# shidanxu/DistributedLPSolver

Measured on AMD Instinct MI355X. Metric: simplex pivots/s + achieved HBM GB/s (dense fp64 tableau; roofline of the rank-64 tableau pass), higher is better.
Workload: dtype f64

## Files before the change

distributedlpsolver_amd/csrc/dlp_pass.hip:

```cpp
#include <hip/hip_runtime.h>

#include <cmath>
#include <cstdlib>
#include <algorithm>
#include <type_traits>
#include <utility>

#include "dlp_host.h"
#include "dlp_internal.h"

namespace dlp {
namespace {

#include "dlp_device.h"
#include "dlp_defer_device.h"

constexpr int kUntouched = -3, kDense = -2, kSparse = -1;

template <int K>
__device__ inline d2 chain_dense(d2 t, const d2* pr, const double* nf) {
#pragma unroll
    for (int l = 0; l < K; ++l) {
        t.x = __builtin_fma(nf[l], pr[l].x, t.x);
        t.y = __builtin_fma(nf[l], pr[l].y, t.y);
// ... 519 lines not shown
#pragma unroll
                for (int u = 0; u < U; ++u)
#pragma unroll
                    for (int e = 0; e < V; ++e)
                        t[u][e] = __builtin_fma(-f[u][l], pr[l0 + l][e], t[u][e]);
    };
    auto grow = [&](int g) { return (int)__builtin_amdgcn_readfirstlane(dgl[g]) * U; };
    const __amdgpu_buffer_rsrc_t rs = __builtin_amdgcn_make_buffer_rsrc(
        (void*)(T + i0 * ld), (short)0, (int)((int64_t)nr * ld * 8), 0x00020000);
    const int voff = (int)(jc * 8);
    const int ld8 = (int)(ld * 8);
    auto load = [&](double (&t)[U][V], int r0) {
#pragma unroll
        for (int u = 0; u < U; ++u) bld<NT, V>(t[u], rs, voff, (r0 + u) * ld8);
    };
    auto store = [&](const double (&t)[U][V], int r0) {
#pragma unroll
        for (int u = 0; u < U; ++u) bst<NT, V>(t[u], rs, voff, (r0 + u) * ld8);
    };
    double fa[U][LC], fb[U][LC];
    auto group_full = [&](double (&t)[U][V], int r0, int rn) {
        const cdptr cb = (cdptr)(cbase + (int64_t)r0 * ldc);
        const cdptr cn = (cdptr)(cbase + (int64_t)rn * ldc);
#pragma unroll
        for (int c = 0; c < NCH; c += 2) {
            __builtin_amdgcn_s_waitcnt(0xC07F);
            fetch(fb, cb, (c + 1) * LC);
            __builtin_amdgcn_sched_barrier(0);
            chain(t, fa, c * LC);
            __builtin_amdgcn_sched_barrier(0);
            __builtin_amdgcn_s_waitcnt(0xC07F);
            if (c + 2 < NCH)
                fetch(fa, cb, (c + 2) * LC);
            else
                fetch(fa, cn, 0);
            __builtin_amdgcn_sched_barrier(0);
            chain(t, fb, (c + 1) * LC);
            __builtin_amdgcn_sched_barrier(0);
        }
        store(t, r0);
    };
    auto group_part = [&](double (&t)[U][V], int r0) {
        const cdptr cb = (cdptr)(cbase + (int64_t)r0 * ldc);
        fetch(fa, cb, 0);
#pragma unroll
        for (int c = 0; c < NCH; c += 2) {
            if (c * LC < kb) {
                __builtin_amdgcn_s_waitcnt(0xC07F);
                if ((c + 1) * LC < kb) fetch(fb, cb, (c + 1) * LC);
                __builtin_amdgcn_sched_barrier(0);
                if ((c + 1) * LC <= kb)
                    chain(t, fa, c * LC);
                else
                    chain_part(t, fa, c * LC);
                __builtin_amdgcn_sched_barrier(0);
                if ((c + 1) * LC < kb) {
                    __builtin_amdgcn_s_waitcnt(0xC07F);
                    if ((c + 2) * LC < kb && c + 2 < NCH) fetch(fa, cb, (c + 2) * LC);
                    __builtin_amdgcn_sched_barrier(0);
                    if ((c + 2) * LC <= kb)
                        chain(t, fb, (c + 1) * LC);
                    else
                        chain_part(t, fb, (c + 1) * LC);
                    __builtin_amdgcn_sched_barrier(0);
                }
            }
        }
        store(t, r0);
    };

    if (ndg > 0) {
        double buf[D][U][V];
#pragma unroll
        for (int b = 0; b < D - 1; ++b) load(buf[b], grow(b < ndg ? b : ndg - 1));
        if constexpr (!PART) fetch(fa, (cdptr)(cbase + (int64_t)grow(0) * ldc), 0);
        for (int g0 = 0; g0 < ndg; g0 += D) {
#pragma unroll
            for (int b = 0; b < D; ++b) {
                const int gi = g0 + b;
                if (gi < ndg) {
                    const int ga = gi + D - 1 < ndg ? gi + D - 1 : ndg - 1;
                    load(buf[(b + D - 1) % D], grow(ga));
                    __builtin_amdgcn_sched_barrier(0);
                    if constexpr (!PART)
                        group_full(buf[b], grow(gi), grow(gi + 1 < ndg ? gi + 1 : gi));
                    else
                        group_part(buf[b], grow(gi));
                }
            }
        }
    }
    for (int r = 0; r < nr; ++r) {
        const int c = cls[r];
        if (c == kUntouched) continue;
        const double* cr = C + (i0 + r) * ldc;
        double t[V];
        int l = 0;
        if (c >= 0) {
            ldrow<false, V>(t, P + (int64_t)c * ld + jc);
            l = c + 1;
        } else {
            bld<NT, V>(t, rs, voff, r * ld8);
        }
        for (; l < kb; ++l) {
            const double f = cr[l];
            if (f != 0.0) {
                double pv[V];
                ldrow<false, V>(pv, P + (int64_t)l * ld + jc);
#pragma unroll
                for (int e = 0; e < V; ++e) t[e] = __builtin_fma(-f, pv[e], t[e]);
            }
        }
        bst<NT, V>(t, rs, voff, r * ld8);
    }
}


constexpr int kDensePiv = 64;
__device__ inline void classify_band(int32_t* cls, const BlockDesc* __restrict__ bd,
                                     const int32_t* __restrict__ nzc, int64_t i0, int nr, int kb,
                                     bool densepiv = false) {
    for (int r = threadIdx.x; r < nr; r += blockDim.x) {
        const int nz = nzc[i0 + r];
        cls[r] = kb == 0 || nz == 0 ? kUntouched : (nz == kb ? kDense : kSparse);
    }
    __syncthreads();
    for (int l = threadIdx.x; l < kb; l += blockDim.x) {
        const int64_t r = (int64_t)bd->pl[l] - i0;
        if (bd->pl[l] >= 0 && r >= 0 && r < nr) atomicMax(&cls[r], l);
    }
    if (!densepiv) return;
    __syncthreads();
    for (int l = threadIdx.x; l < kb; l += blockDim.x) {
        const int64_t r = (int64_t)bd->pl[l] - i0;
        if (bd->pl[l] >= 0 && r >= 0 && r < nr && cls[r] == l && nzc[i0 + r] == kb) cls[r] = kDensePiv + l;
    }
}

template <int N>
__device__ __forceinline__ void fmac_bc(double& t, double c, double p) {
    asm("v_fmac_f64_dpp %0, -%1, %2 row_newbcast:%3 row_mask:0xf bank_mask:0xf"
        : "+v"(t)
        : "v"(c), "v"(p), "n"(N));
}
template <int N>
__device__ __forceinline__ double bc_mov(double v) {
    return __builtin_amdgcn_update_dpp(0.0, v, 0x150 + N, 0xf, 0xf, false);
}
template <int L>
__device__ __forceinline__ void dpp_step(double (&t)[2], const double (&c)[2][2][2], const double (&pr)[64]) {
    constexpr int h = L / 32, e = L & 1, n = (L & 31) >> 1;
    fmac_bc<n>(t[0], c[0][h][e], pr[L]);
    fmac_bc<n>(t[1], c[1][h][e], pr[L]);
}
template <int L0, int... I>
__device__ __forceinline__ void dpp_half(double (&t)[2], const double (&c)[2][2][2], const double (&pr)[64],
                                         std::integer_sequence<int, I...>) {
    (dpp_step<L0 + I>(t, c, pr), ...);
}

template <typename F>
__device__ __forceinline__ double replay_row(double t, int cl, const double (&pr)[64], F f) {
#pragma unroll
    for (int l = 0; l < 64; ++l) {
        const double c = f(l);
        if (l == cl)
            t = pr[l];
        else if (l > cl && c != 0.0)
            t = __builtin_fma(-c, pr[l], t);
    }
    return t;
}

template <bool NT, bool PUB = false>
__global__ __launch_bounds__(256) void pass_d_kernel(const double* __restrict__ T, double* __restrict__ Tout,
                                                     int64_t ld, int64_t rows, int64_t width,
                                                     const BlockDesc* __restrict__ bd,
                                                     const double* __restrict__ C, int64_t ldc,
                                                     const double* __restrict__ P,
                                                     const int32_t* __restrict__ nzc, int rb,
                                                     uint32_t* bcnt = nullptr) {
    constexpr int K = 64, U = 2;
    constexpr int kSt = (NT ? 2 : 0) | (PUB ? kAuxSc1 : 0);
    __shared__ int32_t cls[1024];
    const int kb = bd->blk;
    const bool outplace = Tout != T;
    if (kb == 0 && !outplace) return;
    const int64_t j = (int64_t)blockIdx.x * 256 + threadIdx.x;
    const bool colok = j < width;
    const int jc = (int)(colok ? j : width - 1);
    double pr[K];
#pragma unroll
    for (int l = 0; l < K; ++l) pr[l] = P[(int64_t)l * ld + jc];
    const int64_t i0 = (int64_t)blockIdx.y * rb;
    const int64_t iend = (i0 + rb < rows) ? i0 + rb : rows;
    const int nr = (int)(iend - i0);
    classify_band(cls, bd, nzc, i0, nr, kb);
    __syncthreads();
    const int ld8 = (int)(ld * 8);
    const __amdgpu_buffer_rsrc_t rt = __builtin_amdgcn_make_buffer_rsrc(
        (void*)(T + i0 * ld), (short)0, (int)((int64_t)nr * ld * 8), 0x00020000);
    const __amdgpu_buffer_rsrc_t ro = __builtin_amdgcn_make_buffer_rsrc(
        (void*)(Tout + i0 * ld), (short)0, (int)((int64_t)nr * ld * 8), 0x00020000);
    const __amdgpu_buffer_rsrc_t rc = __builtin_amdgcn_make_buffer_rsrc(
        (void*)(C + i0 * ldc), (short)0, (int)((int64_t)nr * ldc * 8), 0x00020000);
    const int voff = jc * 8;
    const int soff_bad = 0x7fffff00;
    const int voff_st = colok ? voff : soff_bad;
    const int coff = (threadIdx.x & 15) * 16;
    auto dense_at = [&](int r0) {
        if (r0 + U > nr) return false;
        return cls[r0] == kDense && cls[r0 + 1] == kDense;
    };
    double c[U][2][2];
    auto loadc = [&](int r0, int h) {
#pragma unroll
        for (int u = 0; u < U; ++u) {
            const u4v x = __builtin_amdgcn_raw_buffer_load_b128(rc, coff + h * 256, (r0 + u) * (int)ldc * 8, 0);
            const d2 v = __builtin_bit_cast(d2, x);
            c[u][h][0] = v.x;
            c[u][h][1] = v.y;
        }
    };
    auto loadt = [&](double (&t)[U], int r0) {
#pragma unroll
        for (int u = 0; u < U; ++u) {
            const u2v x = __builtin_amdgcn_raw_buffer_load_b64(rt, voff, (r0 + u) * ld8, NT ? 2 : 0);
            t[u] = __builtin_bit_cast(double, x);
        }
    };
    auto group = [&](double (&t)[U], double (&tn)[U], int r0, int rn) {
        loadt(tn, rn);
        __builtin_amdgcn_sched_barrier(0);
        dpp_half<0>(t, c, pr, std::make_integer_sequence<int, 32>{});
        __builtin_amdgcn_sched_barrier(0);
        loadc(rn, 0);
        __builtin_amdgcn_sched_barrier(0);
        dpp_half<32>(t, c, pr, std::make_integer_sequence<int, 32>{});
        __builtin_amdgcn_sched_barrier(0);
        loadc(rn, 1);
        __builtin_amdgcn_sched_barrier(0);
#pragma unroll
        for (int u = 0; u < U; ++u)
            __builtin_amdgcn_raw_buffer_store_b64(__builtin_bit_cast(u2v, t[u]), ro, voff_st, (r0 + u) * ld8,
                                                  kSt);
    };
    double ta[U], tb[U];
    int r = 0;
    while (r < nr) {
        if (dense_at(r)) {
            loadt(ta, r);
            loadc(r, 0);
            loadc(r, 1);
            while (true) {
                const bool nb = dense_at(r + U);
                group(ta, tb, r, nb ? r + U : r);
                r += U;
                if (!nb) break;
                const bool na = dense_at(r + U);
                group(tb, ta, r, na ? r + U : r);
                r += U;
                if (!na) break;
            }
            continue;
        }
        const int cl = cls[r];
        if (cl == kUntouched && outplace) {
            const u2v x = __builtin_amdgcn_raw_buffer_load_b64(rt, voff, r * ld8, NT ? 2 : 0);
            __builtin_amdgcn_raw_buffer_store_b64(x, ro, voff_st, r * ld8, kSt);
        } else if (cl != kUntouched) {
            const double* cr = C + (i0 + r) * ldc;
            double t = 0.0;
            if (cl < 0)
                t = __builtin_bit_cast(double, __builtin_amdgcn_raw_buffer_load_b64(rt, voff, r * ld8, NT ? 2 : 0));
            t = replay_row(t, cl, pr, [&](int l) { return cr[l]; });
            __builtin_amdgcn_raw_buffer_store_b64(__builtin_bit_cast(u2v, t), ro, voff_st, r * ld8, kSt);
        }
        r += 1;
    }
    if constexpr (PUB) {
        asm volatile("s_waitcnt vmcnt(0)" ::: "memory");
        __syncthreads();
        if (threadIdx.x == 0) __hip_atomic_fetch_add(&bcnt[blockIdx.y], 1u, __ATOMIC_RELAXED, __HIP_MEMORY_SCOPE_AGENT);
    }
}

template <int D, int U>
__device__ __forceinline__ void vmwait_group(int g) {
    static_assert(D <= 8 && 2 * U * (D - 1) <= 63, "vmcnt holds 6 bits");
    if (g >= D - 1) {
        vmwait<2 * U * (D - 1)>();
        return;
    }
    switch (g) {
        case 0: vmwait<U * (D - 1)>(); break;
        case 1: vmwait<U * (D - 1) + U>(); break;
        case 2: vmwait<U * (D - 1) + 2 * U>(); break;
        case 3: vmwait<U * (D - 1) + 3 * U>(); break;
        case 4: vmwait<U * (D - 1) + 4 * U>(); break;
        case 5: vmwait<U * (D - 1) + 5 * U>(); break;
        default: vmwait<U * (D - 1) + 6 * U>(); break;
    }
}
template <int U, int L>
__device__ __forceinline__ void ring_step(double (&t)[U], const double (&c)[U][2], const double (&pr)[64]) {
    constexpr int e = L & 1, n = (L & 31) >> 1;
#pragma unroll
    for (int u = 0; u < U; ++u) fmac_bc<n>(t[u], c[u][e], pr[L]);
}
template <int U, int L0, int... I>
__device__ __forceinline__ void ring_half(double (&t)[U], const double (&c)[U][2], const double (&pr)[64],
                                          std::integer_sequence<int, I...>) {
    (ring_step<U, L0 + I>(t, c, pr), ...);
}

template <int L>
__device__ __forceinline__ void redo_step(double& t, const double (&c)[2], const double (&pr)[64], int cl) {
    constexpr int e = L & 1, n = (L & 31) >> 1;
    if (L == cl)
        t = pr[L];
    else if (L > cl)
        fmac_bc<n>(t, c[e], pr[L]);
}
template <int L0, int... I>
__device__ __forceinline__ void redo_half(double& t, const double (&c)[2], const double (&pr)[64], int cl,
                                          std::integer_sequence<int, I...>) {
    (redo_step<L0 + I>(t, c, pr, cl), ...);
}
__device__ __forceinline__ double redo_pivot_row(const double* cr, int cl, const double (&pr)[64]) {
    int lane;
    asm volatile("v_mbcnt_lo_u32_b32 %0, -1, 0\n\tv_mbcnt_hi_u32_b32 %0, -1, %0" : "=v"(lane));
    double t = 0.0;
    if (cl < 32) {
        const d2 v = *(const d2*)(cr + 2 * (lane & 15));
        const double c0[2] = {v.x, v.y};
        redo_half<0>(t, c0, pr, cl, std::make_integer_sequence<int, 32>{});
    }
    const d2 v = *(const d2*)(cr + 32 + 2 * (lane & 15));
    const double c1[2] = {v.x, v.y};
    redo_half<32>(t, c1, pr, cl, std::make_integer_sequence<int, 32>{});
    return t;
}

template <bool NT, int U, int D, bool SA = false, bool PUB = false>
__global__ __launch_bounds__(256) __attribute__((amdgpu_waves_per_eu(3))) void pass_q_kernel(
                                                     const double* __restrict__ T, double* __restrict__ Tout,
                                                     int64_t ld, int64_t rows, int64_t width,
                                                     const BlockDesc* __restrict__ bd,
                                                     const double* __restrict__ C, int64_t ldc,
                                                     const double* __restrict__ P,
                                                     const int32_t* __restrict__ nzc, int rb,
                                                     uint32_t* bcnt = nullptr, int pivg = 0) {
    constexpr int K = 64, SLOT = 128 * U;
    constexpr int kSt = (NT ? 2 : 0) | (PUB ? kAuxSc1 : 0);
    static_assert(U % 2 == 0, "one DMA carries two rows");
    __shared__ __attribute__((aligned(16))) int32_t cls[1024];
    typedef int32_t clsv __attribute__((ext_vector_type(U)));
    extern __shared__ double ring[];
    const int kb = bd->blk;
    const bool outplace = Tout != T;
    if (kb == 0 && !outplace) return;
    const int lane = threadIdx.x & 63;
    const int w = __builtin_amdgcn_readfirstlane(threadIdx.x >> 6);
    const int64_t j = (int64_t)blockIdx.x * 256 + threadIdx.x;
    const bool colok = j < width;
    const int jc = (int)(colok ? j : width - 1);
    double pr[K];
#pragma unroll
    for (int l = 0; l < K; ++l) pr[l] = P[(int64_t)l * ld + jc];
    const int64_t i0 = (int64_t)blockIdx.y * rb;
    const int64_t iend = (i0 + rb < rows) ? i0 + rb : rows;
    const int nr = (int)(iend - i0);
    classify_band(cls, bd, nzc, i0, nr, kb, pivg != 0);
    __syncthreads();
#pragma unroll
    for (int l = 0; l < K; ++l) asm volatile("" ::"v"(pr[l]));
    const int ng = (nr + U - 1) / U;
    const int64_t wc = (int64_t)blockIdx.x * 256 + w * 64 + 2 * (lane & 31);
    const int64_t wcc = wc < ld - 1 ? wc : ld - 2;
    double* wbase = ring + (size_t)w * D * SLOT;
    const uint32_t lbase = (uint32_t)(uintptr_t)(const __attribute__((address_space(3))) void*)wbase;
    uint32_t tvoff = 0, cvoff = 0;
    const double *tsrc = nullptr, *csrc = nullptr;
    if constexpr (SA) {
        tvoff = (uint32_t)(lane >> 5) * (uint32_t)(ld * 8) + (uint32_t)(wcc * 8);
        cvoff = 16u * lane;
    } else {
        tsrc = T + i0 * ld + wcc;
        csrc = C + i0 * ldc + 2 * (lane & 31);
    }
    auto dma = [&](int g, int s) {
        const int gg = g < ng ? g : ng - 1;
#pragma unroll
        for (int k = 0; k < U / 2; ++k) {
            const uint32_t m0 = __builtin_amdgcn_readfirstlane(lbase + s * SLOT * 8 + k * 1024);
            if constexpr (SA) {
                const int rk = gg * U + 2 * k;
                const bool pair = rk + 1 < nr;
                const uint32_t up = lane >> 5 ? (uint32_t)(ld * 8) : 0u;
                glds16s(pair ? tvoff : tvoff - up, T + (i0 + (rk < nr ? rk : nr - 1)) * ld, m0);
            } else {
                int r = gg * U + 2 * k + (lane >> 5);
                r = r < nr ? r : nr - 1;
                glds16(tsrc + (int64_t)r * ld, m0);
            }
        }
#pragma unroll
        for (int k = 0; k < U / 2; ++k) {
            const uint32_t m0 = __builtin_amdgcn_readfirstlane(lbase + s * SLOT * 8 + U * 512 + k * 1024);
            if constexpr (SA) {
                const int rk = gg * U + 2 * k;
                const bool pair = rk + 1 < nr;
                glds16s(pair ? cvoff : cvoff & 511u, C + (i0 + (rk < nr ? rk : nr - 1)) * ldc, m0);
            } else {
                int r = gg * U + 2 * k + (lane >> 5);
                r = r < nr ? r : nr - 1;
                glds16(csrc + (int64_t)r * ldc, m0);
            }
        }
    };
    const int ngs = SA ? nr / U : 0;
    const int64_t tstep = (int64_t)U * ld * 8, cstep = (int64_t)U * ldc * 8;
    const char* tb = (const char*)(T + i0 * ld) + D * tstep;
    const char* cb = (const char*)(C + i0 * ldc) + D * cstep;
    auto dma_s = [&](int s) {
#pragma unroll
        for (int k = 0; k < U / 2; ++k)
            glds16s(tvoff, tb + (int64_t)2 * k * ld * 8,
                    __builtin_amdgcn_readfirstlane(lbase + s * SLOT * 8 + k * 1024));
#pragma unroll
        for (int k = 0; k < U / 2; ++k)
            glds16s(cvoff, cb + (int64_t)2 * k * ldc * 8,
                    __builtin_amdgcn_readfirstlane(lbase + s * SLOT * 8 + U * 512 + k * 1024));
    };
    const int ld8 = (int)(ld * 8);
    const __amdgpu_buffer_rsrc_t ro = __builtin_amdgcn_make_buffer_rsrc(
        (void*)(Tout + i0 * ld), (short)0, (int)((int64_t)nr * ld * 8), 0x00020000);
    const int voff_st = colok ? jc * 8 : 0x7fffff00;
    auto store = [&](double v, int r, bool keep) {
        __builtin_amdgcn_raw_buffer_store_b64(__builtin_bit_cast(u2v, v), ro, keep ? voff_st : 0x7fffff00,
                                              (r < nr ? r : 0) * ld8, kSt);
    };
#pragma unroll
    for (int s = 0; s < D; ++s) dma(s, s);
    int s = 0;
    for (int g = 0; g < ng; ++g) {
        vmwait_group<D, U>(g);
        const double* sl = wbase + s * SLOT;
        const int r0 = g * U;
        const clsv cv = *(const clsv*)(cls + r0);
        bool dense = r0 + U <= nr, anyp = false;
#pragma unroll
        for (int u = 0; u < U; ++u) {
            const int cu = __builtin_amdgcn_readfirstlane(cv[u]);
            dense = dense && (cu == kDense || cu >= kDensePiv);
            anyp = anyp || cu >= kDensePiv;
        }
        if (dense) {
            double t[U];
#pragma unroll
            for (int u = 0; u < U; ++u) t[u] = sl[u * 64 + lane];
            double c[U][2];
            auto loadc = [&](int h) {
#pragma unroll
                for (int u = 0; u < U; ++u) {
                    const d2 v = *(const d2*)(sl + U * 64 + u * 64 + h * 32 + 2 * (lane & 15));
                    c[u][0] = v.x;
                    c[u][1] = v.y;
                }
            };
            loadc(0);
            ring_half<U, 0>(t, c, pr, std::make_integer_sequence<int, 32>{});
            loadc(1);
            ring_half<U, 32>(t, c, pr, std::make_integer_sequence<int, 32>{});
            if (anyp) {
#pragma nounroll
                for (int u = 0; u < U; ++u) {
                    const int cl = __builtin_amdgcn_readfirstlane(cls[r0 + u]) - kDensePiv;
                    if (cl < 0) continue;
                    const double tp = redo_pivot_row(sl + U * 64 + u * 64, cl, pr);
#pragma unroll
                    for (int k = 0; k < U; ++k) t[k] = k == u ? tp : t[k];
                }
            }
#pragma unroll
            for (int u = 0; u < U; ++u) store(t[u], r0 + u, true);
        } else {
            for (int u = 0; u < U; ++u) {
                const int r = r0 + u;
                int cl = r < nr ? cls[r] : kUntouched;
                if (cl >= kDensePiv) cl -= kDensePiv;
                double t = sl[u * 64 + lane];
                if (cl == kUntouched) {
                    store(t, r, outplace && r < nr);
                    continue;
                }
                const double* cr = sl + U * 64 + u * 64;
                t = replay_row(t, cl, pr, [&](int l) { return cr[l]; });
                store(t, r, true);
            }
        }
        if (SA && g + D < ngs) {
            dma_s(s);
        } else {
            dma(g + D, s);
        }
        if constexpr (SA) {
            tb += tstep;
            cb += cstep;
        }
        s = s + 1 == D ? 0 : s + 1;
    }
    if constexpr (PUB) {
        vmwait<0>();
        __syncthreads();
        if (threadIdx.x == 0) __hip_atomic_fetch_add(&bcnt[blockIdx.y], 1u, __ATOMIC_RELAXED, __HIP_MEMORY_SCOPE_AGENT);
    }
}


typedef double d4 __attribute__((ext_vector_type(4)));
template <bool NT_, int NT, bool PUB = false>
__global__ __launch_bounds__(256, 2) void pass_m_kernel(const double* __restrict__ T, double* __restrict__ Tout,
                                                     int64_t ld, int64_t rows, int64_t width,
                                                     const BlockDesc* __restrict__ bd,
                                                     const double* __restrict__ C, int64_t ldc,
                                                     const double* __restrict__ P,
                                                     const int32_t* __restrict__ nzc, int rb,
                                                     uint32_t* bcnt = nullptr) {
    constexpr int kSt = (NT_ ? 2 : 0) | (PUB ? kAuxSc1 : 0);
    constexpr int K = 64, KB = K / 4, W = 16 * NT, RS = K + 2;
    constexpr int NPC = (16 * RS + 127) / 128;
    __shared__ double lds_all[2 * NPC * 128 + 512];
    double(*As)[NPC * 128] = reinterpret_cast<double(*)[NPC * 128]>(lds_all);
    int32_t* cls = reinterpret_cast<int32_t*>(lds_all + 2 * NPC * 128);
    const int kb = bd->blk;
    const bool outplace = Tout != T;
    if (kb == 0 && !outplace) return;
    const int lane = threadIdx.x & 63;
    const int w = __builtin_amdgcn_readfirstlane(threadIdx.x >> 6);
    const int lr = lane & 15, lq = lane >> 4;
    const int64_t cw = (int64_t)blockIdx.x * (4 * W);
    const int64_t c0 = cw + w * W;
    double b[KB][NT];
#pragma unroll
    for (int k4 = 0; k4 < KB; ++k4)
#pragma unroll
        for (int t = 0; t < NT; ++t) {
            const int64_t col = c0 + 16 * t + lr;
            b[k4][t] = P[(int64_t)(4 * k4 + lq) * ld + (col < width ? col : width - 1)];
        }
    const int64_t i0 = (int64_t)blockIdx.y * rb;
    const int64_t iend = (i0 + rb < rows) ? i0 + rb : rows;
    const int nr = (int)(iend - i0);
    classify_band(cls, bd, nzc, i0, nr, kb);
    const int ng = (nr + 15) / 16;
    const int ld8 = (int)(ld * 8);
    const __amdgpu_buffer_rsrc_t ro = __builtin_amdgcn_make_buffer_rsrc(
        (void*)(Tout + i0 * ld), (short)0, (int)((int64_t)nr * ld * 8), 0x00020000);
    (void)ro;
    (void)ld8;
    auto stage = [&](int g, int buf) {
        const int gg = g < ng ? g : ng - 1;
        for (int pc = w; pc < NPC; pc += 4) {
            const int e0 = pc * 128 + 2 * lane;
            int r = e0 / RS, c = e0 % RS;
            if (c >= K || r >= 16) {
                r = 0;
                c = 0;
            }
            int64_t row = i0 + (int64_t)gg * 16 + r;
            row = row < iend ? row : iend - 1;
            __builtin_amdgcn_global_load_lds(C + row * ldc + c,
                                             (__attribute__((address_space(3))) void*)&As[buf][pc * 128], 16, 0, 0);
        }
    };
    auto loadt = [&](d4 (&acc)[NT], int g) {
        const int gg = g < ng ? g : ng - 1;
        const int64_t r0 = i0 + (int64_t)gg * 16;
#pragma unroll
        for (int t = 0; t < NT; ++t) {
            const int64_t col = c0 + 16 * t + lr;
            const int64_t cc = col < width ? col : width - 1;
#pragma unroll
            for (int i = 0; i < 4; ++i) {
                int64_t row = r0 + lq + 4 * i;
                row = row < iend ? row : iend - 1;
                acc[t][i] = NT_ ? __builtin_nontemporal_load(T + row * ld + cc) : T[row * ld + cc];
            }
        }
    };
    d4 ta[NT], tb[NT];
    stage(0, 0);
    loadt(ta, 0);
    constexpr int STG = (NPC + 3) / 4;
    for (int g = 0; g < ng; g += 2) {
#pragma unroll
        for (int h = 0; h < 2; ++h) {
            const int gg = g + h;
            if (gg >= ng) break;
            d4(&acc)[NT] = h == 0 ? ta : tb;
            d4(&nxt)[NT] = h == 0 ? tb : ta;
            asm volatile("s_waitcnt lgkmcnt(0)\n\ts_barrier" ::: "memory");
            stage(gg + 1, (gg + 1) & 1);
            loadt(nxt, gg + 1);
            constexpr int NEWV = NT * 4 + STG;
            __builtin_amdgcn_s_waitcnt(0x3F70 | (NEWV & 0xF) | ((NEWV >> 4) << 14));
            asm volatile("s_barrier" ::: "memory");
            const double* a = &As[gg & 1][lr * RS + lq];
#pragma unroll
            for (int k4 = 0; k4 < KB; ++k4) {
                const double av = -a[4 * k4];
#pragma unroll
                for (int t = 0; t < NT; ++t)
                    acc[t] = __builtin_amdgcn_mfma_f64_16x16x4f64(av, b[k4][t], acc[t], 0, 0, 0);
            }
            const int rl0 = gg * 16;
#pragma unroll
            for (int t = 0; t < NT; ++t) {
                const int64_t col = c0 + 16 * t + lr;
                if (col < width)
#pragma unroll
                    for (int i = 0; i < 4; ++i) {
                        const int rl = rl0 + lq + 4 * i;
                        if (rl < nr && cls[rl] == kDense) {
                            if constexpr (PUB) {
                                const double v = acc[t][i];
                                __builtin_amdgcn_raw_buffer_store_b64(dbits(v), ro,
                                                                      (int)col * 8 + (lq + 4 * i) * ld8, rl0 * ld8,
                                                                      kSt);
                            } else {
                                double* q = Tout + (i0 + rl) * ld + col;
                                if (NT_)
                                    __builtin_nontemporal_store(acc[t][i], q);
                                else
                                    *q = acc[t][i];
                            }
                        }
                    }
            }
        }
    }
    constexpr int WC = 4 * W;
    const int64_t j = cw + (threadIdx.x % WC);
    const bool jok = j < width && threadIdx.x < (256 / WC) * WC;
    for (int r = threadIdx.x / WC; jok && r < nr; r += 256 / WC) {
        const int cl = cls[r];
        if (cl == kDense || (cl == kUntouched && !outplace)) continue;
        const double* row = T + (i0 + r) * ld;
        double t;
        if (cl == kUntouched) {
            t = row[j];
        } else {
            int l = 0;
            if (cl >= 0) {
                t = P[(int64_t)cl * ld + j];
                l = cl + 1;
            } else {
                t = row[j];
            }
            const double* cr = C + (i0 + r) * ldc;
            for (; l < kb; ++l) {
                const double f = cr[l];
                if (f != 0.0) t = __builtin_fma(-f, P[(int64_t)l * ld + j], t);
            }
        }
        if constexpr (PUB)
            __builtin_amdgcn_raw_buffer_store_b64(__builtin_bit_cast(u2v, t), ro, (int)j * 8 + r * ld8, 0, kSt);
        else
            Tout[(i0 + r) * ld + j] = t;
    }
    if constexpr (PUB) {
        asm volatile("s_waitcnt vmcnt(0)" ::: "memory");
        __syncthreads();
        if (threadIdx.x == 0) __hip_atomic_fetch_add(&bcnt[blockIdx.y], 1u, __ATOMIC_RELAXED, __HIP_MEMORY_SCOPE_AGENT);
    }
}

__global__ void blk_reset_kernel(DevState* st) {
    if (threadIdx.x == 0) {
        st->blk = 0;
        st->bser = st->bser + 1;
    }
}

__global__ __launch_bounds__(256) void reset_cols_kernel(double* __restrict__ T, int64_t ld, int64_t rows,
                                                         const int32_t* __restrict__ blkp,
                                                         const int32_t* __restrict__ pl,
                                                         const int32_t* __restrict__ qs) {
    const int64_t i = (int64_t)blockIdx.x * blockDim.x + threadIdx.x;
    if (i >= rows) return;
    const int kb = *blkp;
    double* r = T + i * ld;
    for (int l = 0; l < kb; ++l) r[qs[l]] = (pl[l] == (int32_t)i) ? 1.0 : 0.0;
}

__global__ __launch_bounds__(256) void drop_failed_step_kernel(const DevState* __restrict__ st,
                                                               const int32_t* __restrict__ blkp,
                                                               double* __restrict__ C, int64_t ldc,
                                                               int32_t* __restrict__ nzc, int64_t rows) {
    if (st->status != DLP_UNBOUNDED) return;
    const int kb = *blkp;
    const int64_t i = (int64_t)blockIdx.x * blockDim.x + threadIdx.x;
    if (i > rows || kb < 0 || kb >= ldc) return;
    const double a = C[i * ldc + kb];
    if (i < rows && a != 0.0) nzc[i] = nzc[i] - 1;
    C[i * ldc + kb] = 0.0;
}

__global__ __launch_bounds__(64) void seal_kernel(DevState* st, int slot, uint32_t* bcnt, int64_t nb,
                                                  double* __restrict__ C, int64_t ldc,
                                                  int32_t* __restrict__ nzc, int64_t rows) {
    const int kb = st->blk;
    if (C && nzc && st->status == DLP_UNBOUNDED && kb >= 0 && kb < ldc)
        for (int64_t i = threadIdx.x; i <= rows; i += 64) {
            const double a = C[i * ldc + kb];
            if (i < rows && a != 0.0) nzc[i] = nzc[i] - 1;
            C[i * ldc + kb] = 0.0;
        }
    for (int l = threadIdx.x; l < kMaxDefer; l += 64) {
        st->seal[slot].pl[l] = l < kb ? st->pl[l] : -1;
        st->seal[slot].qs[l] = st->qs[l];
    }
    if (bcnt)
        for (int64_t b = threadIdx.x; b < nb; b += 64) bcnt[b] = 0;
    __syncthreads();
    if (threadIdx.x == 0) {
        st->seal[slot].blk = kb;
        st->seal[slot].ser = st->bser;
        st->blk = 0;
        st->bser = st->bser + 1;
    }
}

}

template <bool NT, int K, int V, int U, int D>
static void launch_pass_r(const Geometry& g, const Defer& d, DevState* st, int rb, size_t dyn,
                          int order, hipStream_t s) {
    const int ntiles = (int)((g.width + 256 * V - 1) / (256 * V));
    const int nbands = (int)((g.rows + rb - 1) / rb);
    const int64_t total = (int64_t)ntiles * nbands;
    const int64_t t8 = (ntiles + 7) / 8;
    const dim3 grid((unsigned)(order == 1 ? 8 * ((total + 7) / 8) : order == 2 ? 8 * t8 * nbands : total));
    pass_r_kernel<NT, K, V, U, D, false><<<grid, 256, dyn, s>>>(
        g.T, g.ld, g.rows, g.width, st, d.C, d.ldc, d.P, d.nzc, rb, ntiles, nbands, order);
    pass_r_kernel<NT, K, V, U, D, true><<<grid, 256, dyn, s>>>(
        g.T, g.ld, g.rows, g.width, st, d.C, d.ldc, d.P, d.nzc, rb, ntiles, nbands, order);
}

static size_t pass_lds_env() {
    static const long v = env_long("DLP_PASS_LDS", 0);
    return v > 0 && v <= 150 * 1024 ? (size_t)v : 0;
}

static bool pass_q_runs(const Geometry& g, const Defer& d, int rb) {
    return d.form == 23 && d.K == 64 && d.ldc == 64 && (int64_t)rb * g.ld * 8 < ((int64_t)1 << 31) && rb <= 1024;
}
static bool pass_saddr_env() {
    static const int v = env_int("DLP_PASS_SADDR", 1);
    return v != 0;
}

static size_t occ_lds(int occ, size_t static_bytes) { return (size_t)160 * 1024 / occ - static_bytes; }
constexpr size_t kClsLds = 1024 * sizeof(int32_t);
constexpr size_t kStreamLds = kClsLds + 512 * sizeof(int16_t) + 16;
constexpr size_t kMfmaLds = kClsLds + 2 * 9 * 128 * sizeof(double);

static bool band_in_descriptor(const Geometry& g, int rb) { return (int64_t)rb * g.ld * 8 < ((int64_t)1 << 31); }

template <bool NT, int U, int D>
static void launch_pass_q(const Geometry& g, const Defer& d, const BlockDesc* bd, double* To, int rb,
                          uint32_t* bcnt, bool sad, int pivg, dim3 grid, size_t dyn, hipStream_t s) {
    auto go = [&](auto sa, auto pub) {
        pass_q_kernel<NT, U, D, decltype(sa)::value, decltype(pub)::value><<<grid, 256, dyn, s>>>(
            g.T, To, g.ld, g.rows, g.width, bd, d.C, d.ldc, d.P, d.nzc, rb, bcnt, pivg);
    };
    constexpr std::true_type yes{};
    constexpr std::false_type no{};
    if (sad)
        bcnt ? go(yes, yes) : go(yes, no);
    else
        bcnt ? go(no, yes) : go(no, no);
}

template <bool NT, int K>
static hipError_t pass(const Geometry& g, const Defer& d, DevState* st, int rb, int occ,
                       hipStream_t s, double* Tout, int seal, uint32_t* bcnt) {
    if (seal >= 0 && !lookahead_form(d.form)) return hipErrorInvalidValue;
    const BlockDesc* bd = seal >= 0 ? &st->seal[seal] : (const BlockDesc*)&st->blk;
    double* To = Tout ? Tout : g.T;
    const unsigned nbands = (unsigned)((g.rows + rb - 1) / rb);
    if (K >= 16 && d.form >= 6 && d.form <= 19 && d.form != 14 && d.form != 15 && band_in_descriptor(g, rb)) {
        if constexpr (K >= 16) {
            if ((d.form == 6 || d.form == 7 || d.form == 10 || d.form == 11 || d.form == 16 ||
                 d.form == 17) && K > 32)
                return hipErrorInvalidValue;
            const size_t dyn = occ > 0 ? occ_lds(occ, kStreamLds) : 0;
            if (g.rows > 0) {
                const int order = d.form <= 9 ? 1 : d.form <= 13 ? 0 : 2;
                const int f = d.form <= 9 ? d.form : d.form <= 13 ? d.form - 4 : d.form - 10;
                if (f == 6) {
                    if constexpr (K <= 32) launch_pass_r<NT, K, 2, 2, 4>(g, d, st, rb, dyn, order, s);
                } else if (f == 7) {
                    if constexpr (K <= 32) launch_pass_r<NT, K, 2, 2, 2>(g, d, st, rb, dyn, order, s);
                } else if (f == 8) {
                    launch_pass_r<NT, K, 1, 4, 4>(g, d, st, rb, dyn, order, s);
                } else {
                    launch_pass_r<NT, K, 1, 4, 2>(g, d, st, rb, dyn, order, s);
                }
            }
        }
    } else if (d.form == 22 && K == 64 && d.K == 64 && d.ldc == 64 && rb <= 1024) {
        if constexpr (K == 64) {
            const size_t dyn = occ > 0 ? occ_lds(occ, kMfmaLds) : 0;
            const dim3 grid((unsigned)((g.width + 127) / 128), nbands);
            if (g.rows > 0) {
                if (bcnt && band_in_descriptor(g, rb))
                    pass_m_kernel<NT, 2, true><<<grid, 256, dyn, s>>>(g.T, To, g.ld, g.rows, g.width, bd, d.C,
                                                                      d.ldc, d.P, d.nzc, rb, bcnt);
                else
                    pass_m_kernel<NT, 2><<<grid, 256, dyn, s>>>(g.T, To, g.ld, g.rows, g.width, bd, d.C, d.ldc,
                                                                 d.P, d.nzc, rb);
            }
        }
    } else if (d.form == 21 && K == 64 && d.K == 64 && d.ldc == 64 && band_in_descriptor(g, rb) &&
               (int64_t)rb * d.ldc * 8 < ((int64_t)1 << 31)) {
        if constexpr (K == 64) {
            const size_t dyn = occ > 0 ? occ_lds(occ, kClsLds) : pass_lds_env();
            const dim3 grid((unsigned)((g.width + 255) / 256), nbands);
            if (g.rows > 0) {
                if (bcnt)
                    pass_d_kernel<NT, true><<<grid, 256, dyn, s>>>(g.T, To, g.ld, g.rows, g.width, bd, d.C, d.ldc,
                                                                   d.P, d.nzc, rb, bcnt);
                else
                    pass_d_kernel<NT><<<grid, 256, dyn, s>>>(g.T, To, g.ld, g.rows, g.width, bd, d.C, d.ldc, d.P,
                                                             d.nzc, rb);
            }
        }
    } else if (K == 64 && pass_q_runs(g, d, rb)) {
        if constexpr (K == 64) {
            static const int qd = env_int("DLP_Q_DEPTH", 4);
            static const int qu_env = env_int("DLP_Q_U", 0);
            static const int pivg = env_int("DLP_PASS_PIVG", 1);
            const bool sad = pass_saddr_env();
            const int U = qu_env == 2 || qu_env == 4 ? qu_env : (g.rows >= 16384 ? 4 : 2);
            const int D = U == 4 ? (qd == 3 ? 3 : 2) : (qd == 2 || qd == 3 || qd == 6 || qd == 8 ? qd : 4);
            size_t dyn = std::max((size_t)4 * D * 128 * U * sizeof(double), pass_lds_env());
            if (occ > 0) dyn = std::max(dyn, occ_lds(occ, kClsLds));
            const dim3 grid((unsigned)((g.width + 255) / 256), nbands);
            if (g.rows <= 0)
                ;
            else if (U == 4 && D == 3)
                launch_pass_q<NT, 4, 3>(g, d, bd, To, rb, bcnt, sad, pivg, grid, dyn, s);
            else if (U == 4)
                launch_pass_q<NT, 4, 2>(g, d, bd, To, rb, bcnt, sad, pivg, grid, dyn, s);
            else if (D == 2)
                launch_pass_q<NT, 2, 2>(g, d, bd, To, rb, bcnt, sad, pivg, grid, dyn, s);
            else if (D == 3)
                launch_pass_q<NT, 2, 3>(g, d, bd, To, rb, bcnt, sad, pivg, grid, dyn, s);
            else if (D == 6)
                launch_pass_q<NT, 2, 6>(g, d, bd, To, rb, bcnt, sad, pivg, grid, dyn, s);
            else if (D == 8)
                launch_pass_q<NT, 2, 8>(g, d, bd, To, rb, bcnt, sad, pivg, grid, dyn, s);
            else
                launch_pass_q<NT, 2, 4>(g, d, bd, To, rb, bcnt, sad, pivg, grid, dyn, s);
        }
    } else {
        const int form = (d.form >= 6 && d.form != 14 && d.form != 15 && d.form != 20) ? 3 : d.form;
        const int cols = (form == 0 || form == 4 || form >= 14) ? kDeferTile : 256;
        const int ntiles = (int)((g.width + cols - 1) / cols);
        const int64_t bands = (g.rows + rb - 1) / rb;
        size_t dyn = form >= 3 ? 0 : (size_t)K * rb * sizeof(double) + (size_t)rb * sizeof(int32_t);
        if (dyn > 160 * 1024) return hipErrorInvalidValue;
        if (occ > 0)
            dyn = std::max(dyn, occ_lds(occ, form >= 14 ? kStreamLds : form >= 3 ? kClsLds : K * sizeof(int32_t)));
        const dim3 grid(ntiles, (unsigned)bands);
        const int tails = d.K == K ? 1 : 0;
        if (g.rows > 0) {
            if (form == 0) {
                if constexpr (K <= 32)
                    pass_kernel<NT, K><<<grid, 256, dyn, s>>>(g.T, g.ld, g.rows, g.width, st, d.C,
                                                              d.ldc, d.P, rb);
                else
                    return hipErrorInvalidValue;
            } else if (form == 3) {
                pass_s_kernel<NT, K, 1, 4, false><<<grid, 256, dyn, s>>>(g.T, To, g.ld, g.rows, g.width, bd,
                                                                         d.C, d.ldc, d.P, d.nzc, rb, tails);
                if (!tails)
                    pass_s_kernel<NT, K, 1, 4, true><<<grid, 256, dyn, s>>>(g.T, To, g.ld, g.rows, g.width, bd,
                                                                            d.C, d.ldc, d.P, d.nzc, rb, 0);
            } else if (form == 20) {
                if constexpr (K <= 32) {
                    pass_s_kernel<NT, K, 2, 2, false, true><<<grid, 256, dyn, s>>>(
                        g.T, To, g.ld, g.rows, g.width, bd, d.C, d.ldc, d.P, d.nzc, rb, tails);
                    if (!tails)
                        pass_s_kernel<NT, K, 2, 2, true><<<grid, 256, dyn, s>>>(
                            g.T, To, g.ld, g.rows, g.width, bd, d.C, d.ldc, d.P, d.nzc, rb, 0);
                } else
                    return hipErrorInvalidValue;
            } else if (form == 4 || form == 14 || form == 15) {
                if constexpr (K <= 32) {
                    const int tl = (form == 14 || form == 15) ? 0 : tails;
                    if (form == 15)
                        pass_s3_kernel<NT, K, 2, 2, false><<<grid, 256, dyn, s>>>(
                            g.T, To, g.ld, g.rows, g.width, bd, d.C, d.ldc, d.P, d.nzc, rb, tl);
                    else
                        pass_s_kernel<NT, K, 2, 2, false><<<grid, 256, dyn, s>>>(
                            g.T, To, g.ld, g.rows, g.width, bd, d.C, d.ldc, d.P, d.nzc, rb, tl);
                    if (form >= 14 && K >= 16 && band_in_descriptor(g, rb)) {
                        const int nb = (int)bands;
                        if constexpr (K >= 16)
                            pass_r_kernel<NT, K, 2, 2, 4, true><<<dim3((unsigned)(ntiles * bands)), 256, dyn, s>>>(
                                g.T, g.ld, g.rows, g.width, st, d.C, d.ldc, d.P, d.nzc, rb, ntiles, nb, 0);
                    } else if (!tl) {
                        pass_s_kernel<NT, K, 2, 2, true><<<grid, 256, dyn, s>>>(
                            g.T, To, g.ld, g.rows, g.width, bd, d.C, d.ldc, d.P, d.nzc, rb, 0);
                    }
                } else
                    return hipErrorInvalidValue;
            } else if (form == 5) {
                pass_s_kernel<NT, K, 1, 8, false><<<grid, 256, dyn, s>>>(g.T, To, g.ld, g.rows, g.width, bd,
                                                                         d.C, d.ldc, d.P, d.nzc, rb, tails);
                if (!tails)
                    pass_s_kernel<NT, K, 1, 8, true><<<grid, 256, dyn, s>>>(g.T, To, g.ld, g.rows, g.width, bd,
                                                                            d.C, d.ldc, d.P, d.nzc, rb, 0);
            }
            else if (form == 1)
                pass1_kernel<NT, K, 2><<<grid, 256, dyn, s>>>(g.T, g.ld, g.rows, g.width, st, d.C,
                                                              d.ldc, d.P, rb);
            else
                pass1_kernel<NT, K, 4><<<grid, 256, dyn, s>>>(g.T, g.ld, g.rows, g.width, st, d.C,
                                                              d.ldc, d.P, rb);
        }
    }
    if (seal < 0) blk_reset_kernel<<<1, 64, 0, s>>>(st);
    return hipGetLastError();
}

template <bool NT>
static hipError_t pass_k(const Geometry& g, const Defer& d, DevState* st, int rb, int occ,
                         hipStream_t s, double* Tout, int seal, uint32_t* bcnt) {
    if (d.K <= 4) return pass<NT, 4>(g, d, st, rb, occ, s, Tout, seal, nullptr);
    if (d.K <= 8) return pass<NT, 8>(g, d, st, rb, occ, s, Tout, seal, nullptr);
    if (d.K <= 16) return pass<NT, 16>(g, d, st, rb, occ, s, Tout, seal, nullptr);
    if (d.K <= 32) return pass<NT, 32>(g, d, st, rb, occ, s, Tout, seal, nullptr);
    return pass<NT, 64>(g, d, st, rb, occ, s, Tout, seal, bcnt);
}

bool lookahead_form(int form) {
    return form == 3 || form == 4 || form == 5 || form == 20 || form == 21 || form == 22 || form == 23;
}

int band_pub_tiles(int form, int64_t width) {
    return (int)(form == 22 ? (width + 127) / 128 : (width + 255) / 256);
}
bool band_pub_ok(const BandPub& bp, const Geometry& g, const Defer& d, int rb) {
    return (d.form == 21 || d.form == 22 || d.form == 23) && d.K == 64 && d.ldc == 64 && rb == bp.rb &&
           (g.rows + rb - 1) / rb <= bp.stride && band_pub_tiles(d.form, g.width) == bp.ntiles &&
           (int64_t)rb * g.ld * 8 < ((int64_t)1 << 31);
}

hipError_t launch_flush_defer(const Geometry& g, const Defer& d, DevState* st, bool nontemporal,
                              int rows_per_block, int occupancy, hipStream_t s, double* Tout,
                              int seal, const BandPub* bp) {
    if (d.K < 1 || d.K > kMaxDefer || rows_per_block < 1 || rows_per_block > 1024 || seal > 1)
        return hipErrorInvalidValue;
    uint32_t* bcnt = nullptr;
    if (bp && bp->cnt && seal >= 0 && Tout && Tout != g.T && band_pub_ok(*bp, g, d, rows_per_block))
        bcnt = bp->cnt + seal * bp->stride;
    if (seal < 0 && g.rows > 0 && d.C && d.nzc) {
        drop_failed_step_kernel<<<(unsigned)((g.rows + 256) / 256), 256, 0, s>>>(st, &st->blk, d.C, d.ldc, d.nzc,
                                                                                g.rows);
        const hipError_t e = hipGetLastError();
        if (e != hipSuccess) return e;
    }
    if (g.cd.on) {
        const hipError_t e = launch_reset_cols(g, st, seal, s);
        if (e != hipSuccess) return e;
    }
    return nontemporal ? pass_k<true>(g, d, st, rows_per_block, occupancy, s, Tout, seal, bcnt)
                       : pass_k<false>(g, d, st, rows_per_block, occupancy, s, Tout, seal, bcnt);
}

hipError_t launch_reset_cols(const Geometry& g, const DevState* st, int seal, hipStream_t s) {
    if (!g.cd.on || g.rows <= 0) return hipSuccess;
    const int32_t* blkp = seal >= 0 ? &st->seal[seal].blk : &st->blk;
    const int32_t* pl = seal >= 0 ? st->seal[seal].pl : st->pl;
    const int32_t* qs = seal >= 0 ? st->seal[seal].qs : st->qs;
    reset_cols_kernel<<<(unsigned)((g.rows + 255) / 256), 256, 0, s>>>(g.T, g.ld, g.rows, blkp, pl, qs);
    return hipGetLastError();
}

hipError_t launch_seal_defer(const Geometry& g, const Defer& d, DevState* st, int slot, hipStream_t s,
                             const BandPub* bp) {
    if (slot < 0 || slot > 1) return hipErrorInvalidValue;
    const bool drop = g.rows > 0 && d.C && d.nzc;
    seal_kernel<<<1, 64, 0, s>>>(st, slot, bp && bp->cnt ? bp->cnt + slot * bp->stride : nullptr,
                                 bp ? bp->stride : 0, drop ? d.C : nullptr, d.ldc, drop ? d.nzc : nullptr, g.rows);
    return hipGetLastError();
}

}
```

Measured before the change: 15070.

## Share C-row staging across waves in the rank-64 pass_q kernel

Adds a CS variant of pass_q_kernel. Instead of each of the four waves loading every C row into its own ring slot, each wave loads one group's C rows into a shared double-buffered LDS ring that all waves read, with an s_barrier every four groups and new counted vmcnt waits. This removes redundant global loads of the C coefficients, which were being fetched four times per block. In exchange it adds a workgroup barrier and a more complex wait schedule, and it is enabled by default only for U=4 with scalar addressing.

```diff
diff --git a/distributedlpsolver_amd/csrc/dlp_pass.hip b/distributedlpsolver_amd/csrc/dlp_pass.hip
--- a/distributedlpsolver_amd/csrc/dlp_pass.hip
+++ b/distributedlpsolver_amd/csrc/dlp_pass.hip
@@ -845,6 +845,24 @@
         default: vmwait<U * (D - 1) + 6 * U>(); break;
     }
 }
+template <int D, int U>
+__device__ __forceinline__ void vmwait_group_cs(int g, int p) {
+    constexpr int h = U / 2;
+    static_assert(D >= 2 && D <= 4 && 3 * h * (D - 1) + h <= 63, "vmcnt holds 6 bits");
+    if (g >= D - 1) {
+        if (p >= 1 && p <= D - 1)
+            vmwait<3 * h * (D - 1) + h>();
+        else
+            vmwait<3 * h * (D - 1)>();
+        return;
+    }
+    if (g == 0)
+        vmwait<h * (D - 1)>();
+    else if (g == 1)
+        vmwait<h * (D > 2 ? D - 2 : 0) + 3 * h + h>();
+    else
+        vmwait<h * (D > 3 ? D - 3 : 0) + 6 * h + h>();
+}
 template <int U, int L>
 __device__ __forceinline__ void ring_step(double (&t)[U], const double (&c)[U][2], const double (&pr)[64]) {
     constexpr int e = L & 1, n = (L & 31) >> 1;
@@ -885,7 +903,7 @@
     return t;
 }
 
-template <bool NT, int U, int D, bool SA = false, bool PUB = false>
+template <bool NT, int U, int D, bool SA = false, bool CS = false, bool PUB = false>
 __global__ __launch_bounds__(256) __attribute__((amdgpu_waves_per_eu(3))) void pass_q_kernel(
                                                      const double* __restrict__ T, double* __restrict__ Tout,
                                                      int64_t ld, int64_t rows, int64_t width,
@@ -894,7 +912,9 @@
                                                      const double* __restrict__ P,
                                                      const int32_t* __restrict__ nzc, int rb,
                                                      uint32_t* bcnt = nullptr, int pivg = 0) {
-    constexpr int K = 64, SLOT = 128 * U;
+    constexpr int K = 64, SLOT = (CS ? 64 : 128) * U;
+    constexpr int G = 4, NS = 2;
+    static_assert(!CS || (SA && G == 4 && D <= G), "one group per wave; the shared ring's counted waits");
     constexpr int kSt = (NT ? 2 : 0) | (PUB ? kAuxSc1 : 0);
     static_assert(U % 2 == 0, "one DMA carries two rows");
     __shared__ __attribute__((aligned(16))) int32_t cls[1024];
@@ -923,6 +943,8 @@
     const int64_t wcc = wc < ld - 1 ? wc : ld - 2;
     double* wbase = ring + (size_t)w * D * SLOT;
     const uint32_t lbase = (uint32_t)(uintptr_t)(const __attribute__((address_space(3))) void*)wbase;
+    const double* cring = ring + (size_t)4 * D * SLOT;
+    const uint32_t cbase = (uint32_t)(uintptr_t)(const __attribute__((address_space(3))) void*)cring;
     uint32_t tvoff = 0, cvoff = 0;
     const double *tsrc = nullptr, *csrc = nullptr;
     if constexpr (SA) {
@@ -948,6 +970,7 @@
                 glds16(tsrc + (int64_t)r * ld, m0);
             }
         }
+        if constexpr (CS) return;
 #pragma unroll
         for (int k = 0; k < U / 2; ++k) {
             const uint32_t m0 = __builtin_amdgcn_readfirstlane(lbase + s * SLOT * 8 + U * 512 + k * 1024);
@@ -971,10 +994,28 @@
         for (int k = 0; k < U / 2; ++k)
             glds16s(tvoff, tb + (int64_t)2 * k * ld * 8,
                     __builtin_amdgcn_readfirstlane(lbase + s * SLOT * 8 + k * 1024));
+        if constexpr (CS) return;
 #pragma unroll
         for (int k = 0; k < U / 2; ++k)
             glds16s(cvoff, cb + (int64_t)2 * k * ldc * 8,
                     __builtin_amdgcn_readfirstlane(lbase + s * SLOT * 8 + U * 512 + k * 1024));
+    };
+    auto dma_c = [&](int sg, int cs) {
+        const int gq = G * sg + w;
+        const uint32_t dst = cbase + (uint32_t)((cs * G + w) * U * 512);
+        const bool inside = (gq + 1) * U <= nr;
+        const int gg = gq < ng ? gq : ng - 1;
+#pragma unroll
+        for (int k = 0; k < U / 2; ++k) {
+            const uint32_t m0 = __builtin_amdgcn_readfirstlane(dst + k * 1024);
+            if (inside) {
+                glds16s(cvoff, C + (i0 + gq * U + 2 * k) * ldc, m0);
+            } else {
+                const int rk = gg * U + 2 * k;
+                const bool pair = rk + 1 < nr;
+                glds16s(pair ? cvoff : cvoff & 511u, C + (i0 + (rk < nr ? rk : nr - 1)) * ldc, m0);
+            }
+        }
     };
     const int ld8 = (int)(ld * 8);
     const __amdgpu_buffer_rsrc_t ro = __builtin_amdgcn_make_buffer_rsrc(
@@ -984,12 +1025,23 @@
         __builtin_amdgcn_raw_buffer_store_b64(__builtin_bit_cast(u2v, v), ro, keep ? voff_st : 0x7fffff00,
                                               (r < nr ? r : 0) * ld8, kSt);
     };
+    if constexpr (CS) dma_c(0, 0);
 #pragma unroll
     for (int s = 0; s < D; ++s) dma(s, s);
     int s = 0;
     for (int g = 0; g < ng; ++g) {
-        vmwait_group<D, U>(g);
+        if constexpr (CS) {
+            const int p = g % G;
+            vmwait_group_cs<D, U>(g, p);
+            if (p == 0) {
+                asm volatile("s_barrier" ::: "memory");
+                dma_c(g / G + 1, (g / G + 1) % NS);
+            }
+        } else {
+            vmwait_group<D, U>(g);
+        }
         const double* sl = wbase + s * SLOT;
+        const double* cf = CS ? cring + g % (NS * G) * U * 64 : sl + U * 64;
         const int r0 = g * U;
         const clsv cv = *(const clsv*)(cls + r0);
         bool dense = r0 + U <= nr, anyp = false;
@@ -1007,7 +1059,7 @@
             auto loadc = [&](int h) {
 #pragma unroll
                 for (int u = 0; u < U; ++u) {
-                    const d2 v = *(const d2*)(sl + U * 64 + u * 64 + h * 32 + 2 * (lane & 15));
+                    const d2 v = *(const d2*)(cf + u * 64 + h * 32 + 2 * (lane & 15));
                     c[u][0] = v.x;
                     c[u][1] = v.y;
                 }
@@ -1021,7 +1073,7 @@
                 for (int u = 0; u < U; ++u) {
                     const int cl = __builtin_amdgcn_readfirstlane(cls[r0 + u]) - kDensePiv;
                     if (cl < 0) continue;
-                    const double tp = redo_pivot_row(sl + U * 64 + u * 64, cl, pr);
+                    const double tp = redo_pivot_row(cf + u * 64, cl, pr);
 #pragma unroll
                     for (int k = 0; k < U; ++k) t[k] = k == u ? tp : t[k];
                 }
@@ -1038,7 +1090,7 @@
                     store(t, r, outplace && r < nr);
                     continue;
                 }
-                const double* cr = sl + U * 64 + u * 64;
+                const double* cr = cf + u * 64;
                 t = replay_row(t, cl, pr, [&](int l) { return cr[l]; });
                 store(t, r, true);
             }
@@ -1312,19 +1364,36 @@
 
 static bool band_in_descriptor(const Geometry& g, int rb) { return (int64_t)rb * g.ld * 8 < ((int64_t)1 << 31); }
 
+static int pass_cshare_env() {
+    static const int v = env_int("DLP_PASS_CSHARE", -1);
+    return v;
+}
+static bool pass_cshare_default(int U) { return U == 4; }
+constexpr bool pass_q_shared_exists(int U, int D) { return (U == 4 && (D == 2 || D == 3)) || (U == 2 && D == 4); }
+constexpr int kCsG = 4, kCsNS = 2;
+static size_t pass_q_lds(int U, int D, bool shared) {
+    return shared ? ((size_t)4 * D + kCsNS * kCsG) * 64 * U * sizeof(double) : (size_t)4 * D * 128 * U * sizeof(double);
+}
+
 template <bool NT, int U, int D>
 static void launch_pass_q(const Geometry& g, const Defer& d, const BlockDesc* bd, double* To, int rb,
-                          uint32_t* bcnt, bool sad, int pivg, dim3 grid, size_t dyn, hipStream_t s) {
-    auto go = [&](auto sa, auto pub) {
-        pass_q_kernel<NT, U, D, decltype(sa)::value, decltype(pub)::value><<<grid, 256, dyn, s>>>(
-            g.T, To, g.ld, g.rows, g.width, bd, d.C, d.ldc, d.P, d.nzc, rb, bcnt, pivg);
+                          uint32_t* bcnt, bool sad, bool csh, int pivg, dim3 grid, size_t dyn, hipStream_t s) {
+    auto go = [&](auto sa, auto cs, auto pub) {
+        pass_q_kernel<NT, U, D, decltype(sa)::value, decltype(cs)::value, decltype(pub)::value>
+            <<<grid, 256, dyn, s>>>(g.T, To, g.ld, g.rows, g.width, bd, d.C, d.ldc, d.P, d.nzc, rb, bcnt, pivg);
     };
     constexpr std::true_type yes{};
     constexpr std::false_type no{};
+    if constexpr (pass_q_shared_exists(U, D)) {
+        if (sad && csh) {
+            bcnt ? go(yes, yes, yes) : go(yes, yes, no);
+            return;
+        }
+    }
     if (sad)
-        bcnt ? go(yes, yes) : go(yes, no);
+        bcnt ? go(yes, no, yes) : go(yes, no, no);
     else
-        bcnt ? go(no, yes) : go(no, no);
+        bcnt ? go(no, no, yes) : go(no, no, no);
 }
 
 template <bool NT, int K>
@@ -1389,25 +1458,27 @@
             const bool sad = pass_saddr_env();
             const int U = qu_env == 2 || qu_env == 4 ? qu_env : (g.rows >= 16384 ? 4 : 2);
             const int D = U == 4 ? (qd == 3 ? 3 : 2) : (qd == 2 || qd == 3 || qd == 6 || qd == 8 ? qd : 4);
-            size_t dyn = std::max((size_t)4 * D * 128 * U * sizeof(double), pass_lds_env());
+            const int cse = pass_cshare_env();
+            const bool csh = sad && pass_q_shared_exists(U, D) && (cse >= 0 ? cse != 0 : pass_cshare_default(U));
+            size_t dyn = std::max(pass_q_lds(U, D, csh), pass_lds_env());
             if (occ > 0) dyn = std::max(dyn, occ_lds(occ, kClsLds));
             const dim3 grid((unsigned)((g.width + 255) / 256), nbands);
             if (g.rows <= 0)
                 ;
             else if (U == 4 && D == 3)
-                launch_pass_q<NT, 4, 3>(g, d, bd, To, rb, bcnt, sad, pivg, grid, dyn, s);
+                launch_pass_q<NT, 4, 3>(g, d, bd, To, rb, bcnt, sad, csh, pivg, grid, dyn, s);
             else if (U == 4)
-                launch_pass_q<NT, 4, 2>(g, d, bd, To, rb, bcnt, sad, pivg, grid, dyn, s);
+                launch_pass_q<NT, 4, 2>(g, d, bd, To, rb, bcnt, sad, csh, pivg, grid, dyn, s);
             else if (D == 2)
-                launch_pass_q<NT, 2, 2>(g, d, bd, To, rb, bcnt, sad, pivg, grid, dyn, s);
+                launch_pass_q<NT, 2, 2>(g, d, bd, To, rb, bcnt, sad, csh, pivg, grid, dyn, s);
             else if (D == 3)
-                launch_pass_q<NT, 2, 3>(g, d, bd, To, rb, bcnt, sad, pivg, grid, dyn, s);
+                launch_pass_q<NT, 2, 3>(g, d, bd, To, rb, bcnt, sad, csh, pivg, grid, dyn, s);
             else if (D == 6)
-                launch_pass_q<NT, 2, 6>(g, d, bd, To, rb, bcnt, sad, pivg, grid, dyn, s);
+                launch_pass_q<NT, 2, 6>(g, d, bd, To, rb, bcnt, sad, csh, pivg, grid, dyn, s);
             else if (D == 8)
-                launch_pass_q<NT, 2, 8>(g, d, bd, To, rb, bcnt, sad, pivg, grid, dyn, s);
+                launch_pass_q<NT, 2, 8>(g, d, bd, To, rb, bcnt, sad, csh, pivg, grid, dyn, s);
             else
-                launch_pass_q<NT, 2, 4>(g, d, bd, To, rb, bcnt, sad, pivg, grid, dyn, s);
+                launch_pass_q<NT, 2, 4>(g, d, bd, To, rb, bcnt, sad, csh, pivg, grid, dyn, s);
         }
     } else {
         const int form = (d.form >= 6 && d.form != 14 && d.form != 15 && d.form != 20) ? 3 : d.form;
```

After: 15260 (median of 6 runs). +1.2%, better.
